# bentherien/point-cloud-reid

Hardware: AMD Instinct MI355X
Metric: siamese pair-comparisons/sec @1024 pts (higher is better)
Workload: dtype bf16x3

## Files before the change

point-cloud-reid_amd/csrc/attn_kernels_impl.h:

```cpp
#pragma once
#ifndef PCR_ATTN_PREC
#define PCR_ATTN_PREC 0
#endif
#include "tile_dense.h"
#include "wave_trace.h"

#include <stdio.h>

#include <initializer_list>
#include <vector>

namespace {
constexpr int kAPrec = PCR_ATTN_PREC;
struct AttnArgs {
  pcr_attn_params p;
  int dbg;
  int wpc;
  const int *live_count;
  int live_period, live_offset;
};

struct LiveWalk {
  unsigned n, period;
  long total;
  __device__ __forceinline__ long map(long v) const {
    const unsigned q = (unsigned)v / n;
    return (long)q * period + ((unsigned)v - q * n);
  }
};
__device__ __forceinline__ unsigned live_pairs(const AttnArgs &a) {
  int c = __builtin_amdgcn_readfirstlane(*a.live_count);
  c = c < 0 ? 0 : c;
  c -= a.live_offset;
  return (unsigned)(c < 0 ? 0 : (c > a.live_period ? a.live_period : c));
}
__device__ __forceinline__ LiveWalk live_walk(const AttnArgs &a) {
  LiveWalk w;
  w.n = live_pairs(a);
  w.period = (unsigned)a.live_period;
  const unsigned B = (unsigned)a.p.B, full = B / w.period, rem = B - full * w.period;
  w.total = (long)full * w.n + (rem < w.n ? rem : w.n);
  return w;
}
__device__ __forceinline__ bool live_cloud(const AttnArgs &a, unsigned b) {
  return b % (unsigned)a.live_period < live_pairs(a);
}

constexpr int kATraceWgs = 512, kATraceRecs = 24, kATraceMarks = 8;
using AttnTrace = WaveTrace<0, kATraceRecs, kATraceMarks, 2 * kATraceWgs>;
__device__ unsigned long long g_attn_trace[AttnTrace::kCap * AttnTrace::kWords];


__device__ __forceinline__ void pos_hidden(float *dst, int RP, const float *P, const float *w0,
                                           const float *b0, int d, int T) {
  for (int e = threadIdx.x; e < d * T; e += blockDim.x) {
    const int o = e / T, t = e - o * T;
    const float v = w0[o * 3] * P[t] + w0[o * 3 + 1] * P[RP + t] + w0[o * 3 + 2] * P[2 * RP + t] + b0[o];
    dst[o * RP + t] = fmaxf(v, 0.f);
  }
}

__device__ __forceinline__ void load_xyz3(float *P, int RP, const float *xyz, int L, int t0, int T) {
  for (int e = threadIdx.x; e < 3 * T; e += blockDim.x) {
    const int c = e / T, t = e - c * T;
    P[c * RP + t] = t0 + t < L ? xyz[(size_t)(t0 + t) * 3 + c] : 0.f;
  }
}

__device__ __forceinline__ void attn_kv_fold_write(const pcr_attn_params &p, const float *KVl, const float *s_kt, size_t b) {
  const int d = p.d, dh = d / p.nhead, ld = d + 1, tid = threadIdx.x;
  float *kv = p.kv + b * ((size_t)d * d + d);
  const int d_o = kThreads / d, d_dd = kThreads - d_o * d;
  int o = tid / d, dd = tid - o * d;
  int v0 = (dd / dh) * dh;
  for (int e = tid; e < d * d; e += kThreads, o += d_o, dd += d_dd) {
    if (dd >= d) {
      dd -= d;
      o++;
    }
    if (d_dd) v0 = (dd / dh) * dh;
    const float *wm = p.wmerge + (size_t)o * d + v0;
    const float *kr = KVl + dd * ld + v0;
    float m = 0.f;
#pragma unroll 8
    for (int v = 0; v < dh; v++) m += wm[v] * kr[v];
    if constexpr (kAPrec == 0) {
      const int kb = dd >> 3, rem = dd & 7;
      kv[(((size_t)kb * d + o) * 2 + (rem & 1)) * 4 + (rem >> 1)] = m;
    } else {
      const int s16 = dd >> 4, kk = dd & 15;
      const int hh = (kk >> 2) & 1, jj = (kk & 3) + ((kk >> 3) << 2);
      const size_t unit = (((size_t)s16 * (d >> 5) + (o >> 5)) * 2) * 64 + hh * 32 + (o & 31);
      const __bf16 hi = (__bf16)m;
      const __bf16 lo = (__bf16)(m - (float)hi);
      __bf16 *img = reinterpret_cast<__bf16 *>(kv);
      img[unit * 8 + jj] = hi;
      img[(unit + 64) * 8 + jj] = lo;
    }
  }
  __syncthreads();
  if (tid < d) kv[(size_t)d * d + tid] = s_kt[tid];
}

__device__ __forceinline__ void attn_kv_fold_mfma(const pcr_attn_params &p, const float *KVt, const float *s_kt, size_t b) {
  const int d = p.d, dh = d / p.nhead, ld = d + 1, tid = threadIdx.x;
  float *kv = p.kv + b * ((size_t)d * d + d);
  for (int hd = 0; hd < p.nhead; hd++) {
    const float *wm = p.wmerge_packed + (size_t)(hd * dh / 8) * d * 8;
    tile_dense(KVt + (size_t)(hd * dh) * ld + hd * dh, dh, ld, dh >> 5, wm, d, [&](float m, int o, int t) {
      const int dd = hd * dh + t;
      if constexpr (kAPrec == 0) {
        const int kb = dd >> 3, rem = dd & 7;
        kv[(((size_t)kb * d + o) * 2 + (rem & 1)) * 4 + (rem >> 1)] = m;
      } else {
        const int s16 = dd >> 4, kk = dd & 15;
        const int hh = (kk >> 2) & 1, jj = (kk & 3) + ((kk >> 3) << 2);
        const size_t unit = (((size_t)s16 * (d >> 5) + (o >> 5)) * 2) * 64 + hh * 32 + (o & 31);
        const __bf16 hi = (__bf16)m;
        const __bf16 lo = (__bf16)(m - (float)hi);
        __bf16 *img = reinterpret_cast<__bf16 *>(kv);
        img[unit * 8 + jj] = hi;
        img[(unit + 64) * 8 + jj] = lo;
      }
    });
  }
  __syncthreads();
  if (tid < d) kv[(size_t)d * d + tid] = s_kt[tid];
}

template <int TB, int NR, int WSEL, int NTW, bool BFP = false>
__device__ __forceinline__ void attn_kv_body(const AttnArgs &a) {
  constexpr int T = 32 * TB, RP = T + 1;
  constexpr int NPF = 4;
  extern __shared__ __attribute__((aligned(16))) float smem[];
  const pcr_attn_params &p = a.p;
  const int d = p.d, c2 = p.c2;
  float *XH = smem;
  float *KB = XH;
  float *VB = XH + d * RP;
  float *P = XH + (c2 + d) * RP;
  float *s_w0 = P + 3 * RP, *s_b0 = s_w0 + 3 * d;
  const int tail_a = (c2 + d + 3) * RP + 4 * d, tail_b = d * (d + 1) + d;
  float *s_ks = smem + (tail_a > tail_b ? tail_a : tail_b);
  const int tid = threadIdx.x, lane = tid & 63, wave = tid >> 6;
  const int l31 = lane & 31, h = lane >> 5;
  const size_t b = blockIdx.x;
  for (int e = tid; e < 3 * d; e += kThreads) s_w0[e] = p.pos0_w[e];
  for (int e = tid; e < d; e += kThreads) s_b0[e] = p.pos0_b[e];
  const float *feat = p.feat_k + b * c2 * p.Sk;
  const float *xyz = p.xyz_k + b * p.Sk * 3;
  const int nb = d >> 5, nT = nb * nb;
  const int dh = d / p.nhead;
  const float sk = (float)p.Sk;
  const float *bkv = p.bkv;

  f32x16 acc[NTW];
#pragma unroll
  for (int i = 0; i < NTW; i++)
#pragma unroll
    for (int r = 0; r < 16; r++) acc[i][r] = 0.f;
  int tile_ib[NTW];
#pragma unroll
// ... 28 lines not shown
        dst[2] = pf[u][2];
        dst[3] = pf[u][3];
      }
    }
  };
  const int nsplit = p.kv_splits > 1 ? p.kv_splits : 1;
  const int ntile = (p.Sk + T - 1) / T, tps = (ntile + nsplit - 1) / nsplit;
  const int t_lo = (int)blockIdx.y * tps * T;
  const int t_hi = (t_lo + tps * T) < p.Sk ? (t_lo + tps * T) : p.Sk;
  bool have = false;
  if (vec_ok && t_lo + T <= p.Sk && t_lo < t_hi) {
    fetch(t_lo);
    have = true;
  }
  for (int t0 = t_lo; t0 < t_hi; t0 += T) {
    const int valid = p.Sk - t0;
    if (have) stash();
    else load_tile(XH, RP, feat, c2, c2, p.Sk, t0, T);
    load_xyz3(P, RP, xyz, p.Sk, t0, T);
    __syncthreads();
    have = vec_ok && t0 + 2 * T <= p.Sk && t0 + T < t_hi;
    pos_hidden(XH + c2 * RP, RP, P, s_w0, s_b0, d, T);
    __syncthreads();
    auto kv_epi = [&](const f32x16 &acc, int cb, int tb, int l31, int h) {
      const int t = tb * 32 + l31;
      float *dst = XH + (cb * 32 + 4 * h) * RP + t;
      const bool live = t < valid;
      if (cb * 32 < d) {
#pragma unroll
        for (int r = 0; r < 16; r++) dst[((r & 3) + 8 * (r >> 2)) * RP] = live ? elu1(acc[r]) : 0.f;
      } else {
#pragma unroll
        for (int r = 0; r < 16; r++) dst[((r & 3) + 8 * (r >> 2)) * RP] = live ? acc[r] / sk : 0.f;
      }
    };
    auto kv_hook = [&]() { if (have) fetch(t0 + T); };
    if constexpr (BFP && kAPrec != 0 && WSEL != 0)
      tile_dense2p<kAPrec, TB, NR, WSEL, true>(XH, c2 + d, p.wkv_bf, 2 * d, true, kv_epi, bkv, nullptr, kv_hook);
    else
      tile_dense2<TB, NR, WSEL, true>(XH, c2 + d, p.wkv, 2 * d, true, kv_epi, bkv, nullptr, kv_hook);
    __syncthreads();
    {
      const float *row = KB + krow * RP;
      for (int t = kpart; t < T; t += kparts) ksum += row[t];
    }
#pragma unroll
    for (int it = 0; it < NTW; it++) {
      const int item = wave + 4 * it;
      if (item < nT) {
        const int ib = tile_ib[it], jb = item - ib * nb;
        const float *ap = KB + (ib * 32 + l31) * RP + h;
        const float *bp = VB + (jb * 32 + l31) * RP + h;
#pragma unroll 4
        for (int ks = 0; ks < T / 2; ks++)
          acc[it] = __builtin_amdgcn_mfma_f32_32x32x2f32(ap[2 * ks], bp[2 * ks], acc[it], 0, 0, 0);
      }
    }
    __syncthreads();
  }
  if (nsplit > 1) {
    float *part = p.kv_part + ((size_t)b * nsplit + blockIdx.y) * ((size_t)d * d + d);
    s_ks[tid] = ksum;
#pragma unroll
    for (int it = 0; it < NTW; it++) {
      const int item = wave + 4 * it;
      if (item < nT) {
        const int ib = tile_ib[it], jb = item - ib * nb;
#pragma unroll
        for (int r = 0; r < 16; r++)
          part[(size_t)(ib * 32 + (r & 3) + 8 * (r >> 2) + 4 * h) * d + jb * 32 + l31] = acc[it][r];
      }
    }
    __syncthreads();
    if (tid < d) {
      float s = 0.f;
      for (int pp = 0; pp < kparts; pp++) s += s_ks[pp * d + tid];
      part[(size_t)d * d + tid] = s;
    }
    return;
  }
  float *KVl = smem;
  const int ld = d + 1;
  const bool mfma_fold = p.wmerge_packed != nullptr && (dh & 31) == 0 && (d & 31) == 0;
  float *s_kt = smem + d * ld;
  s_ks[tid] = ksum;
#pragma unroll
  for (int it = 0; it < NTW; it++) {
    const int item = wave + 4 * it;
    if (item < nT) {
      const int ib = tile_ib[it], jb = item - ib * nb;
      const int v = jb * 32 + l31;
      const int hv = v / dh;
      const bool aligned = (dh & 31) == 0;
      const bool same_blk = (ib * 32) / dh == hv;
#pragma unroll
      for (int r = 0; r < 16; r++) {
        const int dd = ib * 32 + (r & 3) + 8 * (r >> 2) + 4 * h;
        const bool same = aligned ? same_blk : (dd / dh == hv);
        if (mfma_fold) KVl[v * ld + dd] = same ? acc[it][r] : 0.f;
        else KVl[dd * ld + v] = same ? acc[it][r] : 0.f;
      }
    }
  }
  __syncthreads();
  if (tid < d) {
    float s = 0.f;
    for (int pp = 0; pp < kparts; pp++) s += s_ks[pp * d + tid];
    s_kt[tid] = s;
  }
  if (mfma_fold) attn_kv_fold_mfma(p, KVl, s_kt, b);
  else attn_kv_fold_write(p, KVl, s_kt, b);
}

template <int TB, int NR, int WSEL, int NTW>
__global__ __launch_bounds__(kThreads) void attn_kv_kernel(AttnArgs a) {
  attn_kv_body<TB, NR, WSEL, NTW>(a);
}
template <int TB, int NR, int WSEL, int NTW>
__global__ __launch_bounds__(kThreads) __attribute__((amdgpu_waves_per_eu(3, 3))) void attn_kv_kernel_o3(AttnArgs a) {
  attn_kv_body<TB, NR, WSEL, NTW>(a);
}
template <int TB, int NR, int WSEL, int NTW>
__global__ __launch_bounds__(kThreads) __attribute__((amdgpu_waves_per_eu(3, 3))) void attn_kv_kernel_o3_live(AttnArgs a) {
  if (!live_cloud(a, blockIdx.x)) return;
  attn_kv_body<TB, NR, WSEL, NTW>(a);
}
template <int TB, int NR, int WSEL, int NTW, bool BFP = false>
__global__ __launch_bounds__(kThreads) __attribute__((amdgpu_waves_per_eu(2, 2))) void attn_kv_kernel_o2(AttnArgs a) {
  attn_kv_body<TB, NR, WSEL, NTW, BFP>(a);
}

constexpr int kKvsWaves = 8;
template <bool DIAG, bool BF, int XS = 4, bool ONEW = false, bool GATE = false>
__global__ __launch_bounds__(64 * kKvsWaves) __attribute__((amdgpu_waves_per_eu(2, 2)))
void attn_kv_stream64_kernel(AttnArgs a) {
  static_assert(BF || XS == 4, "the f32 form is c2 = 64 only");
  constexpr int D = 64, LD = D + 1, KVS = D * LD + D;
  constexpr int NKV = DIAG ? 2 : 4;
  constexpr int C2 = 16 * XS, WU = BF ? (XS + 4) * 512 : 4096, MINW = XS == 8 ? 4 : 2;
  extern __shared__ __attribute__((aligned(16))) float smem[];
  const pcr_attn_params &p = a.p;
  f32x4 *s_w = reinterpret_cast<f32x4 *>(smem);
  f32x4 *s_p0 = reinterpret_cast<f32x4 *>(smem + 4 * WU);
  float *s_bkv = smem + 4 * WU + 256;
  float *s_wm = s_bkv + 128;
  float *s_red = s_wm + D * LD;
  const int tid = threadIdx.x, lane = tid & 63, j = lane & 31, h = lane >> 5;
  const int wave = __builtin_amdgcn_readfirstlane(tid >> 6);
  LiveWalk lw{};
  if constexpr (GATE) {
    lw = live_walk(a);
    if ((long)blockIdx.x * (kKvsWaves / (ONEW ? 1 : 4)) >= lw.total) return;
  }
  {
    const f32x4 *src = reinterpret_cast<const f32x4 *>(BF ? p.wkv_bf : p.wkv);
    for (int e = tid; e < WU; e += 64 * kKvsWaves) s_w[e] = src[e];
    for (int e = tid; e < D * D; e += 64 * kKvsWaves) s_wm[(e >> 6) * LD + (e & 63)] = p.wmerge[e];
    if (tid < D) s_p0[tid] = f32x4{p.pos0_w[3 * tid], p.pos0_w[3 * tid + 1], p.pos0_w[3 * tid + 2], p.pos0_b[tid]};
    if (tid < 2 * D) s_bkv[tid] = p.bkv[tid];
  }
  __syncthreads();
  const int nblk = p.Sk >> 5;
  constexpr int kMaxWpc = 4;
  const int wpc = nblk < kMaxWpc ? nblk : kMaxWpc;
  int wpc2 = 1;
  while (wpc2 * 2 <= wpc) wpc2 *= 2;
  if (wpc2 < MINW) wpc2 = MINW;
  if constexpr (ONEW) wpc2 = 1;
  const int cpg = kKvsWaves / wpc2;
  const int cslot = wave / wpc2, wsub = wave - cslot * wpc2;
  const float inv_sk = 1.0f / (float)p.Sk;
  float bias[4];
#pragma unroll
  for (int cb = 0; cb < 4; cb++) bias[cb] = s_bkv[cb * 32 + j];
  const int dh = D / p.nhead;
  AttnTrace trace;
  if constexpr (kTraceBuild)
    trace.begin((a.dbg & 256) && lane == 0 && (wave == 0 || wave == 5) && blockIdx.x < kATraceWgs,
                g_attn_trace, 2 * blockIdx.x + (wave ? 1 : 0));
  const long nB = GATE ? lw.total : (long)p.B;
  for (long c0 = (long)blockIdx.x * cpg; c0 < nB; c0 += (long)gridDim.x * cpg) {
    const bool live = c0 + cslot < nB;
    const long b = GATE ? (live ? lw.map(c0 + cslot) : 0) : c0 + cslot;
    trace.mark(4);
    f32x16 kv[NKV];
#pragma unroll
    for (int i = 0; i < NKV; i++)
#pragma unroll
      for (int r = 0; r < 16; r++) kv[i][r] = 0.f;
    float ks0 = 0.f, ks1 = 0.f;
    if (live) {
      const float *feat = p.feat_k + (size_t)b * C2 * p.Sk;
      const float *xyz = p.xyz_k + (size_t)b * p.Sk * 3;
      const __amdgpu_buffer_rsrc_t rfeat =
          __builtin_amdgcn_make_buffer_rsrc(const_cast<float *>(feat), 0, C2 * p.Sk * 4, 0x00020000);
      for (int blk = wsub; blk < nblk; blk += wpc2) {
        asm volatile("" ::: "memory");
        trace.mark(0);
        const int t = blk * 32 + j;
        const float px = xyz[3 * t], py = xyz[3 * t + 1], pz = xyz[3 * t + 2];
        f32x16 acc[4];
        if constexpr (!BF) {
          float xr[64];
          {
            const int vo = (h * p.Sk + t) * 4;
#pragma unroll
            for (int s2 = 0; s2 < 32; s2++)
              xr[s2] = __builtin_bit_cast(float, __builtin_amdgcn_raw_buffer_load_b32(rfeat, vo, s2 * 2 * p.Sk * 4, 0));
          }
#pragma unroll
          for (int s2 = 0; s2 < 32; s2++) {
            const f32x4 w = s_p0[2 * s2 + h];
            const float v = w[0] * px + w[1] * py + w[2] * pz + w[3];
            xr[32 + s2] = fmaxf(v, 0.f);
          }
#pragma unroll
          for (int s2 = 0; s2 < 32; s2++) asm volatile("" : "+v"(xr[s2]));
#pragma unroll
          for (int cb = 0; cb < 4; cb++)
#pragma unroll
            for (int r = 0; r < 16; r++) acc[cb][r] = 0.f;
#pragma unroll
          for (int kb = 0; kb < 16; kb++) {
            f32x4 w[4];
#pragma unroll
            for (int cb = 0; cb < 4; cb++) w[cb] = s_w[((kb * 128 + cb * 32 + j) << 1) + h];
#pragma unroll
            for (int i = 0; i < 4; i++)
#pragma unroll
              for (int cb = 0; cb < 4; cb++)
                acc[cb] = __builtin_amdgcn_mfma_f32_32x32x2f32(xr[4 * kb + i], w[cb][i], acc[cb], 0, 0, 0);
          }
        } else {
          float xf[8 * XS];
          {
            const int vo = (4 * h * p.Sk + t) * 4;
#pragma unroll
            for (int e = 0; e < 8 * XS; e++) {
              const int ch = 16 * (e >> 3) + bf_kpos(0, e & 7);
              xf[e] = __builtin_bit_cast(float, __builtin_amdgcn_raw_buffer_load_b32(rfeat, vo, ch * p.Sk * 4, 0));
            }
          }
          bf16x8 ah[XS + 4], al[XS + 4];
#pragma unroll
          for (int s2 = 0; s2 < 4; s2++) {
            float hv[8];
#pragma unroll
            for (int e = 0; e < 8; e++) {
              const f32x4 w = s_p0[16 * s2 + bf_kpos(0, e) + 4 * h];
              const float v = w[0] * px + w[1] * py + w[2] * pz + w[3];
              hv[e] = relu_i(v);
            }
            bf_split8(hv, ah[XS + s2], al[XS + s2], true);
          }
#pragma unroll
          for (int e = 0; e < 8 * XS; e++) asm volatile("" : "+v"(xf[e]));
#pragma unroll
          for (int s2 = 0; s2 < XS; s2++) {
            float xv[8];
#pragma unroll
            for (int e = 0; e < 8; e++) xv[e] = xf[8 * s2 + e];
            bf_split8(xv, ah[s2], al[s2], true);
          }
#pragma unroll
          for (int cb = 0; cb < 4; cb++)
#pragma unroll
            for (int r = 0; r < 16; r++) acc[cb][r] = 0.f;
          trace.mark(1);
          const bf16x8 *wb = reinterpret_cast<const bf16x8 *>(s_w) + lane;
#pragma unroll
          for (int s2 = 0; s2 < XS + 4; s2++) {
            bf16x8 wh[4], wl[4];
#pragma unroll
            for (int cb = 0; cb < 4; cb++) {
              wh[cb] = wb[((s2 * 4 + cb) * 2) * 64];
              wl[cb] = wb[((s2 * 4 + cb) * 2 + 1) * 64];
            }
#pragma unroll
            for (int cb = 0; cb < 4; cb++) acc[cb] = __builtin_amdgcn_mfma_f32_32x32x16_bf16(ah[s2], wh[cb], acc[cb], 0, 0, 0);
#pragma unroll
            for (int cb = 0; cb < 4; cb++) acc[cb] = __builtin_amdgcn_mfma_f32_32x32x16_bf16(al[s2], wh[cb], acc[cb], 0, 0, 0);
#pragma unroll
            for (int cb = 0; cb < 4; cb++) acc[cb] = __builtin_amdgcn_mfma_f32_32x32x16_bf16(ah[s2], wl[cb], acc[cb], 0, 0, 0);
          }
        }
        trace.mark(2);
#pragma unroll
        for (int r = 0; r < 16; r++) {
          acc[0][r] = elu1(acc[0][r] + bias[0]);
          acc[1][r] = elu1(acc[1][r] + bias[1]);
          acc[2][r] = (acc[2][r] + bias[2]) * inv_sk;
          acc[3][r] = (acc[3][r] + bias[3]) * inv_sk;
          ks0 += acc[0][r];
          ks1 += acc[1][r];
        }
#pragma unroll
        for (int i = 0; i < NKV; i++) {
          const int ib = DIAG ? i : (i >> 1), jb = DIAG ? i : (i & 1);
#pragma unroll
          for (int r = 0; r < 16; r++) {
            if constexpr (ONEW) kv[i] = __builtin_amdgcn_mfma_f32_32x32x2f32(acc[2 + jb][r], acc[ib][r], kv[i], 0, 0, 0);
            else kv[i] = __builtin_amdgcn_mfma_f32_32x32x2f32(acc[ib][r], acc[2 + jb][r], kv[i], 0, 0, 0);
          }
        }
        trace.mark(3);
      }
    }
    trace.mark(5);
    ks0 += __shfl_xor(ks0, 32, 64);
    ks1 += __shfl_xor(ks1, 32, 64);
    if constexpr (ONEW) {
      if (live) {
        float *kvo = p.kv + (size_t)b * ((size_t)D * D + D);
        bf16x8 *img = reinterpret_cast<bf16x8 *>(kvo);
#pragma unroll
        for (int db = 0; db < 2; db++) {
          const int hd = (db * 32 + j) / dh;
#pragma unroll
          for (int ob = 0; ob < 2; ob++) {
            f32x16 m;
#pragma unroll
            for (int r = 0; r < 16; r++) m[r] = 0.f;
#pragma unroll
            for (int i = 0; i < NKV; i++) {
              const int ib = DIAG ? i : (i >> 1), jb = DIAG ? i : (i & 1);
              if (ib != db) continue;
              const float *wr = s_wm + (ob * 32 + j) * LD + jb * 32 + 4 * h;
#pragma unroll
              for (int r = 0; r < 16; r++) {
                const int vl = (r & 3) + 8 * (r >> 2);
                const float av = (jb * 32 + vl + 4 * h) / dh == hd ? kv[i][r] : 0.f;
                m = __builtin_amdgcn_mfma_f32_32x32x2f32(av, wr[vl], m, 0, 0, 0);
              }
            }
#pragma unroll
            for (int G = 0; G < 2; G++) {
              float v[8];
#pragma unroll
              for (int e = 0; e < 8; e++) v[e] = m[8 * G + e];
              bf16x8 hi, lo;
              bf_split8(v, hi, lo, true);
              const size_t unit = (((size_t)(db * 2 + G) * (D >> 5) + ob) * 2) * 64 + h * 32 + j;
              img[unit] = hi;
              img[unit + 64] = lo;
            }
          }
        }
        if (h == 0) {
          kvo[(size_t)D * D + j] = ks0;
          kvo[(size_t)D * D + 32 + j] = ks1;
        }
      }
      trace.mark(6);
      trace.mark(7);
      trace.next();
      continue;
    }
    float *KVl = s_red + cslot * KVS, *s_kt = KVl + D * LD;
    for (int round = 0; round < wpc2; round++) {
      if (wsub == round) {
#pragma unroll
        for (int i = 0; i < NKV; i++) {
          const int ib = DIAG ? i : (i >> 1), jb = DIAG ? i : (i & 1);
#pragma unroll
          for (int r = 0; r < 16; r++) {
            const int dd = ib * 32 + (r & 3) + 8 * (r >> 2) + 4 * h, v = jb * 32 + j;
            float *dst = KVl + dd * LD + v;
            *dst = round == 0 ? kv[i][r] : *dst + kv[i][r];
          }
        }
        if (h == 0) {
          s_kt[j] = round == 0 ? ks0 : s_kt[j] + ks0;
          s_kt[32 + j] = round == 0 ? ks1 : s_kt[32 + j] + ks1;
        }
      }
      __syncthreads();
    }
    trace.mark(6);
    if (live) {
      float *kvo = p.kv + (size_t)b * ((size_t)D * D + D);
      for (int ti = wsub; ti < 4; ti += wpc2) {
        const int ob = ti >> 1, db = ti & 1;
        const float *ap = s_wm + (ob * 32 + j) * LD + h;
        const float *bp = KVl + (db * 32 + j) * LD + h;
        const int hd = (db * 32 + j) / dh;
        f32x16 m;
#pragma unroll
        for (int r = 0; r < 16; r++) m[r] = 0.f;
        const int s_lo = DIAG ? db * 16 : 0, s_hi = DIAG ? db * 16 + 16 : 32;
        if constexpr (kAPrec == 0) {
#pragma unroll 4
          for (int s2 = s_lo; s2 < s_hi; s2++) {
            const float bv = bp[2 * s2];
            m = __builtin_amdgcn_mfma_f32_32x32x2f32(ap[2 * s2], (2 * s2 + h) / dh == hd ? bv : 0.f, m, 0, 0, 0);
          }
          const int dd = db * 32 + j;
#pragma unroll
          for (int r = 0; r < 16; r++) {
            const int o = ob * 32 + (r & 3) + 8 * (r >> 2) + 4 * h;
            const int kb = dd >> 3, rem = dd & 7;
            kvo[(((size_t)kb * D + o) * 2 + (rem & 1)) * 4 + (rem >> 1)] = m[r];
          }
        } else {
#pragma unroll 4
          for (int s2 = s_lo; s2 < s_hi; s2++) {
            const float bv = bp[2 * s2];
            m = __builtin_amdgcn_mfma_f32_32x32x2f32((2 * s2 + h) / dh == hd ? bv : 0.f, ap[2 * s2], m, 0, 0, 0);
          }
          bf16x8 *img = reinterpret_cast<bf16x8 *>(kvo);
#pragma unroll
          for (int G = 0; G < 2; G++) {
            float v[8];
#pragma unroll
            for (int e = 0; e < 8; e++) v[e] = m[8 * G + e];
            bf16x8 hi, lo;
            bf_split8(v, hi, lo, true);
            const size_t unit = (((size_t)(db * 2 + G) * (D >> 5) + ob) * 2) * 64 + h * 32 + j;
            img[unit] = hi;
            img[unit + 64] = lo;
          }
        }
      }
      for (int e = wsub * 64 + lane; e < D; e += 64 * wpc2) kvo[(size_t)D * D + e] = s_kt[e];
    }
    trace.mark(7);
    trace.next();
    __syncthreads();
  }
}

#if PCR_ATTN_PREC != 0
__global__ __launch_bounds__(64 * kKvsWaves) __attribute__((amdgpu_waves_per_eu(2, 4)))
void attn_kv_stream32_kernel(AttnArgs a) {
  constexpr int D = 32, LD = D + 1, KVS = D * LD + D;
  extern __shared__ __attribute__((aligned(16))) float smem[];
  const pcr_attn_params &p = a.p;
// ... 1502 lines not shown
  const bool wide = 2 * p.d > 128 || p.cout > 128 || p.cfinal > 128;
  if (tb == 4) return attn_plan_form(pl, PCR_ATTN_APPLY_TILE, {4, wide ? 2 : 1}, false, gated);
  if (tb == 2) return attn_plan_form(pl, PCR_ATTN_APPLY_TILE, {2, wide ? 2 : 1}, true, gated);
  int widest = 2 * p.d > p.cout ? 2 * p.d : p.cout;
  if (p.cfinal > widest) widest = p.cfinal;
  if (kAPrec != 0 && widest > 256) return PCR_ERR_INVALID;
  return attn_plan_form(pl, PCR_ATTN_APPLY_TILE, {1, widest > 512 ? 8 : (widest > 256 ? 4 : 2)}, false, gated);
}

static dim3 attn_grid(const AttnPlan &pl) {
  if (!pl.persistent) return dim3(pl.gx, pl.gy);
  const long cap = (long)pl.per_cu * pcr_cu_count();
  return dim3((unsigned)(pl.work < cap ? pl.work : cap));
}
template <auto KERN, auto KERN_LIVE>
static inline int attn_launch_g(const AttnPlan &pl, dim3 grid, hipStream_t st, const AttnArgs &a) {
  return pl.gated ? pcr_launch_lds<KERN_LIVE>(grid, dim3(pl.threads), pl.lds, st, a)
                  : pcr_launch_lds<KERN>(grid, dim3(pl.threads), pl.lds, st, a);
}

static int attn_launch_kv_tile(const AttnPlan &pl, const AttnArgs &a, hipStream_t st) {
  const dim3 g = attn_grid(pl), blk(pl.threads);
  if (pl.targ[0] == 2) return pcr_launch_lds<attn_kv_kernel<2, 1, 2, 1>>(g, blk, pl.lds, st, a);
  return pcr_launch_lds<attn_kv_kernel<1, 2, 0, 4>>(g, blk, pl.lds, st, a);
}
static int attn_launch_kv_tile_o3(const AttnPlan &pl, const AttnArgs &a, hipStream_t st) {
  return attn_launch_g<attn_kv_kernel_o3<2, 1, 1, 1>, attn_kv_kernel_o3_live<2, 1, 1, 1>>(pl, attn_grid(pl), st, a);
}
static int attn_launch_kv_tile_o2(const AttnPlan &pl, const AttnArgs &a, hipStream_t st) {
  const dim3 g = attn_grid(pl), blk(pl.threads);
  if (pl.targ[4]) return pcr_launch_lds<attn_kv_kernel_o2<1, 2, 1, 4, true>>(g, blk, pl.lds, st, a);
  return pcr_launch_lds<attn_kv_kernel_o2<1, 2, 1, 4>>(g, blk, pl.lds, st, a);
}
template <bool DIAG>
static int attn_launch_kv_stream64(const AttnPlan &pl, const AttnArgs &a, const AttnTune &t, hipStream_t st) {
  const dim3 g = attn_grid(pl);
  int rc = PCR_ERR_INVALID;
  if (!pl.targ[1])
    rc = attn_launch_g<attn_kv_stream64_kernel<DIAG, false>, attn_kv_stream64_kernel<DIAG, false, 4, false, true>>(pl, g, st, a);
#if PCR_ATTN_PREC != 0
  else if (pl.targ[2] == 8) rc = pcr_launch_lds<attn_kv_stream64_kernel<DIAG, true, 8>>(g, dim3(pl.threads), pl.lds, st, a);
  else if (pl.targ[3])
    rc = attn_launch_g<attn_kv_stream64_kernel<DIAG, true, 4, true>, attn_kv_stream64_kernel<DIAG, true, 4, true, true>>(pl, g, st, a);
  else rc = attn_launch_g<attn_kv_stream64_kernel<DIAG, true>, attn_kv_stream64_kernel<DIAG, true, 4, false, true>>(pl, g, st, a);
#endif
  if (pl.trace) attn_dump_trace(t.trace, "kv64", (int)g.x, (int)a.p.B, a.p.Sk);
  return rc;
}
#if PCR_ATTN_PREC != 0
static int attn_launch_kv_stream32(const AttnPlan &pl, const AttnArgs &a, hipStream_t st) {
  return pcr_launch_lds<attn_kv_stream32_kernel>(attn_grid(pl), dim3(pl.threads), pl.lds, st, a);
}
static int attn_launch_kv_stream128(const AttnPlan &pl, const AttnArgs &a, hipStream_t st) {
  const dim3 g = attn_grid(pl), blk(pl.threads);
  if (pl.targ[0] == 2) return pcr_launch_lds<attn_kv_stream128_kernel<2>>(g, blk, pl.lds, st, a);
  return pcr_launch_lds<attn_kv_stream128_kernel<4>>(g, blk, pl.lds, st, a);
}
#else
static int attn_launch_kv_wide(const AttnPlan &pl, const AttnArgs &a, hipStream_t st) {
  const dim3 g = attn_grid(pl), blk(pl.threads);
  if (pl.targ[0] == 2) return pcr_launch_lds<attn_kv_wide_kernel<2>>(g, blk, pl.lds, st, a);
  return pcr_launch_lds<attn_kv_wide_kernel<3>>(g, blk, pl.lds, st, a);
}
#endif

static int attn_launch_kv(const AttnPlan &pl, AttnArgs &a, const AttnTune &t, hipStream_t st) {
  int rc = PCR_ERR_INVALID;
  if (pl.family != PCR_ATTN_KV_WIDE) a.p.kv_splits = pl.splits;
  switch (pl.family) {
    case PCR_ATTN_KV_TILE: rc = attn_launch_kv_tile(pl, a, st); break;
    case PCR_ATTN_KV_TILE_O3: rc = attn_launch_kv_tile_o3(pl, a, st); break;
    case PCR_ATTN_KV_TILE_O2: rc = attn_launch_kv_tile_o2(pl, a, st); break;
    case PCR_ATTN_KV_STREAM64:
      return pl.targ[0] ? attn_launch_kv_stream64<true>(pl, a, t, st) : attn_launch_kv_stream64<false>(pl, a, t, st);
#if PCR_ATTN_PREC != 0
    case PCR_ATTN_KV_STREAM32: return attn_launch_kv_stream32(pl, a, st);
    case PCR_ATTN_KV_STREAM128: return attn_launch_kv_stream128(pl, a, st);
#else
    case PCR_ATTN_KV_WIDE: return attn_launch_kv_wide(pl, a, st);
#endif
    default: return PCR_ERR_INVALID;
  }
  if (rc != PCR_OK || !pl.fold) return rc;
  return pcr_launch_lds<attn_kv_fold_kernel>(dim3(a.p.B), dim3(pl.threads), pl.fold_lds, st, a);
}

static int attn_launch_apply_tile(const AttnPlan &pl, const AttnArgs &a, hipStream_t st) {
  const dim3 g = attn_grid(pl), blk(pl.threads);
  switch (pl.targ[0] * 10 + pl.targ[1]) {
    case 41: return pcr_launch_lds<attn_apply_kernel<4, 1>>(g, blk, pl.lds, st, a);
    case 42: return pcr_launch_lds<attn_apply_kernel<4, 2>>(g, blk, pl.lds, st, a);
    case 21: return attn_launch_g<attn_apply_kernel<2, 1>, attn_apply_kernel<2, 1, true>>(pl, g, st, a);
    case 22: return attn_launch_g<attn_apply_kernel<2, 2>, attn_apply_kernel<2, 2, true>>(pl, g, st, a);
    case 12: return pcr_launch_lds<attn_apply_kernel<1, 2>>(g, blk, pl.lds, st, a);
#if PCR_ATTN_PREC == 0
    case 14: return pcr_launch_lds<attn_apply_kernel<1, 4>>(g, blk, pl.lds, st, a);
    case 18: return pcr_launch_lds<attn_apply_kernel<1, 8>>(g, blk, pl.lds, st, a);
#endif
    default: return PCR_ERR_INVALID;
  }
}
#if PCR_ATTN_PREC != 0
template <bool QPOS>
static int attn_launch_apply_stream64(const AttnPlan &pl, const AttnArgs &a, const AttnTune &t, hipStream_t st) {
  const dim3 g = attn_grid(pl), blk(pl.threads);
  const int c1s = pl.targ[1], cf = pl.targ[2], nob = pl.targ[3], nd = pl.targ[4];
  int rc = PCR_ERR_INVALID;
  if (nd == 1) rc = pcr_launch_lds<attn_apply_stream64_kernel<QPOS, 2, 0, 1, 1>>(g, blk, pl.lds, st, a);
  else if (nob == 4) rc = pcr_launch_lds<attn_apply_stream64_kernel<QPOS, 4, 0, 4>>(g, blk, pl.lds, st, a);
  else if (c1s == 4 && cf && !pl.targ[5])
    rc = attn_launch_g<attn_apply_stream64_kernel<QPOS, 4, 4>, attn_apply_stream64_kernel<QPOS, 4, 4, 2, 2, false, true>>(pl, g, st, a);
  else if (c1s == 4 && !pl.targ[5])
    rc = attn_launch_g<attn_apply_stream64_kernel<QPOS, 4, 0>, attn_apply_stream64_kernel<QPOS, 4, 0, 2, 2, false, true>>(pl, g, st, a);
  else if constexpr (!QPOS) {
    if (pl.targ[5])
      return attn_launch_g<attn_apply_stream64_kernel<false, 4, 0, 2, 2, true>, attn_apply_stream64_kernel<false, 4, 0, 2, 2, true, true>>(pl, g, st, a);
    if (c1s == 1) rc = pcr_launch_lds<attn_apply_stream64_kernel<false, 1, 2, 1>>(g, blk, pl.lds, st, a);
    else if (cf) rc = pcr_launch_lds<attn_apply_stream64_kernel<false, 2, 4>>(g, blk, pl.lds, st, a);
    else rc = pcr_launch_lds<attn_apply_stream64_kernel<false, 2, 0>>(g, blk, pl.lds, st, a);
  }
  if (pl.trace) attn_dump_trace(t.trace, "apply64", (int)g.x, (int)a.p.B, a.p.Lq);
  return rc;
}
static int attn_launch_apply_stream128(const AttnPlan &pl, const AttnArgs &a, hipStream_t st) {
  const dim3 g = attn_grid(pl), blk(pl.threads);
  if (pl.targ[0] == 1) return pcr_launch_lds<attn_apply_stream128_kernel<1>>(g, blk, pl.lds, st, a);
  if (pl.targ[0] == 2) return pcr_launch_lds<attn_apply_stream128_kernel<2>>(g, blk, pl.lds, st, a);
  return pcr_launch_lds<attn_apply_stream128_kernel<4>>(g, blk, pl.lds, st, a);
}
#endif

static int attn_launch_apply(const AttnPlan &pl, const AttnArgs &a, const AttnTune &t, hipStream_t st) {
  (void)t;
  switch (pl.family) {
    case PCR_ATTN_APPLY_TILE: return attn_launch_apply_tile(pl, a, st);
#if PCR_ATTN_PREC != 0
    case PCR_ATTN_APPLY_STREAM64:
      return pl.targ[0] ? attn_launch_apply_stream64<true>(pl, a, t, st) : attn_launch_apply_stream64<false>(pl, a, t, st);
    case PCR_ATTN_APPLY_STREAM128: return attn_launch_apply_stream128(pl, a, st);
#endif
    default: return PCR_ERR_INVALID;
  }
}

static int attn_unit(const pcr_attn_params &p, const pcr_live *live, bool apply, AttnPlan *pl, bool launch, pcr_stream_t stream) {
  const AttnTune &t = attn_tune();
  *pl = AttnPlan();
  const int rc = apply ? attn_plan_apply(p, live != nullptr, t, pl) : attn_plan_kv(p, live != nullptr, t, pl);
  if (!launch) return rc;
  if (pl->arith >= 0) pcr_note_arith(pl->arith);
  if (rc != PCR_OK) return rc;
  AttnArgs a;
  a.p = p;
  a.dbg = pl->trace ? 256 : 0;
  a.wpc = pl->wpc;
  a.live_count = live ? live->count : nullptr;
  a.live_period = live ? live->period : 0;
  a.live_offset = live ? live->offset : 0;
  return apply ? attn_launch_apply(*pl, a, t, pcr_s(stream)) : attn_launch_kv(*pl, a, t, pcr_s(stream));
}

#if PCR_ATTN_PREC == 1
int pcr_attn_kv_bf3(const pcr_attn_params *pp, const pcr_live *live, AttnPlan *pl, bool launch, pcr_stream_t stream) {
  return attn_unit(*pp, live, false, pl, launch, stream);
}
int pcr_attn_apply_bf3(const pcr_attn_params *pp, const pcr_live *live, AttnPlan *pl, bool launch, pcr_stream_t stream) {
  return attn_unit(*pp, live, true, pl, launch, stream);
}
#else
int pcr_attn_kv_bf3(const pcr_attn_params *pp, const pcr_live *live, AttnPlan *pl, bool launch, pcr_stream_t stream);
int pcr_attn_apply_bf3(const pcr_attn_params *pp, const pcr_live *live, AttnPlan *pl, bool launch, pcr_stream_t stream);

static bool attn_bf(const pcr_attn_params &p, pcr_attn_params &q) {
  const int widest = 2 * p.d > p.cout ? (2 * p.d > p.cfinal ? 2 * p.d : p.cfinal) : (p.cout > p.cfinal ? p.cout : p.cfinal);
  if (p.precision == 0 || p.d > 128 || widest > 256 || !p.wq_bf || !p.wmlp0_bf || !p.wmlp2_bf ||
      (p.cfinal && !p.wfinal_bf))
    return false;
  q = p;
  q.wq = p.wq_bf; q.wmlp0 = p.wmlp0_bf; q.wmlp2 = p.wmlp2_bf; q.wfinal = p.wfinal_bf;
  return true;
}

PCR_EXPORT int pcr_attn_kv_splits(int B, int Sk, int d) {
  (void)B;
  if (Sk < 1 || d > 64) return 1;
  if ((d == 64 || d == 32) && (Sk & 31) == 0) return 1;
  const int ntile = (Sk + 63) / 64;
  return ntile >= 16 ? 4 : (ntile >= 8 ? 2 : 1);
}

static bool attn_pool_ok(const pcr_attn_params &p) {
  pcr_attn_params q;
  return aps64_shape(p) && p.c1 == 64 && p.cout == 64 && !p.cfinal && !p.q_pos && attn_bf(p, q);
}

static int attn_entry(const pcr_attn_params *pp, const pcr_live *live, bool apply, AttnPlan *pl, bool launch, pcr_stream_t stream) {
  if (!pp || attn_check(*pp)) return PCR_ERR_INVALID;
  if (apply && ((!pp->out && !pp->pool_out) || (pp->pool_out && !attn_pool_ok(*pp)))) return PCR_ERR_INVALID;
  if (live && !attn_live_shape(*pp)) return PCR_ERR_INVALID;
  if (launch && pp->B == 0) return PCR_OK;
  if (apply && pp->B > 65535) return PCR_ERR_INVALID;
  if (live && (!live->count || live->period < 1 || live->offset < 0)) return PCR_ERR_INVALID;
  pcr_attn_params q;
  if (attn_bf(*pp, q)) return apply ? pcr_attn_apply_bf3(&q, live, pl, launch, stream) : pcr_attn_kv_bf3(&q, live, pl, launch, stream);
  return attn_unit(*pp, live, apply, pl, launch, stream);
}

PCR_EXPORT int pcr_attn_kv_f32(const pcr_attn_params *pp, pcr_stream_t stream) {
  AttnPlan pl;
  return attn_entry(pp, nullptr, false, &pl, true, stream);
}
PCR_EXPORT int pcr_attn_kv_live_f32(const pcr_attn_params *pp, const pcr_live *live, pcr_stream_t stream) {
  AttnPlan pl;
  return attn_entry(pp, live, false, &pl, true, stream);
}
PCR_EXPORT int pcr_attn_apply_f32(const pcr_attn_params *pp, pcr_stream_t stream) {
  AttnPlan pl;
  return attn_entry(pp, nullptr, true, &pl, true, stream);
}
PCR_EXPORT int pcr_attn_apply_live_f32(const pcr_attn_params *pp, const pcr_live *live, pcr_stream_t stream) {
  AttnPlan pl;
  return attn_entry(pp, live, true, &pl, true, stream);
}
PCR_EXPORT int pcr_attn_live_ok(const pcr_attn_params *pp) {
  return (pp && !attn_check(*pp) && attn_live_shape(*pp)) ? 1 : 0;
}
PCR_EXPORT int pcr_attn_apply_pool_ok(const pcr_attn_params *pp) {
  return (pp && !attn_check(*pp) && attn_pool_ok(*pp)) ? 1 : 0;
}

PCR_EXPORT int pcr_attn_launch_form(const pcr_attn_params *pp, const pcr_live *live, int apply, int *form) {
  if (!form) return PCR_ERR_INVALID;
  AttnPlan pl;
  const int rc = attn_entry(pp, live, apply != 0, &pl, false, nullptr);
  if (rc != PCR_OK) return rc;
  for (int i = 0; i < PCR_ATTN_FORM_INTS; i++) form[i] = 0;
  form[0] = pl.arith;
  form[1] = pl.family;
  form[2] = pl.gated;
  form[3] = pl.ntarg;
  for (int i = 0; i < pl.ntarg; i++) form[4 + i] = pl.targ[i];
  if (!apply) {
    form[10] = pl.splits;
    form[11] = pl.fold;
    form[12] = pl.wpc;
  }
  form[13] = (int)pl.lds;
  return PCR_OK;
}
#endif
```

Before: 69640.

## Skip zero key-weight blocks for positional channels in KV projection

```diff
diff --git a/point-cloud-reid_amd/csrc/attn_kernels_impl.h b/point-cloud-reid_amd/csrc/attn_kernels_impl.h
--- a/point-cloud-reid_amd/csrc/attn_kernels_impl.h
+++ b/point-cloud-reid_amd/csrc/attn_kernels_impl.h
@@ -8,6 +8,7 @@
 #include <stdio.h>
 
 #include <initializer_list>
+#include <type_traits>
 #include <vector>
 
 namespace {
@@ -342,14 +343,28 @@
     lw = live_walk(a);
     if ((long)blockIdx.x * (kKvsWaves / (ONEW ? 1 : 4)) >= lw.total) return;
   }
+  static_assert(LD > D, "s_kz takes the pad column of s_wm's last row");
+  unsigned *s_kz = reinterpret_cast<unsigned *>(s_wm + (D - 1) * LD + D);
+  if (tid == 0) *s_kz = 0u;
+  __syncthreads();
   {
     const f32x4 *src = reinterpret_cast<const f32x4 *>(BF ? p.wkv_bf : p.wkv);
-    for (int e = tid; e < WU; e += 64 * kKvsWaves) s_w[e] = src[e];
+    unsigned nz = 0u;
+    for (int e = tid; e < WU; e += 64 * kKvsWaves) {
+      const f32x4 u = src[e];
+      s_w[e] = u;
+      const bool kz = BF ? ((e >> 9) >= XS && ((e >> 7) & 3) < 2) : ((e >> 8) >= 8 && ((e >> 1) & 127) < D);
+      typedef unsigned u32x4 __attribute__((ext_vector_type(4)));
+      const u32x4 ub = __builtin_bit_cast(u32x4, u);
+      if (kz) nz |= (ub[0] | ub[1] | ub[2] | ub[3]) & (BF ? 0x7FFF7FFFu : 0x7FFFFFFFu);
+    }
+    if (nz) atomicOr(s_kz, 1u);
     for (int e = tid; e < D * D; e += 64 * kKvsWaves) s_wm[(e >> 6) * LD + (e & 63)] = p.wmerge[e];
     if (tid < D) s_p0[tid] = f32x4{p.pos0_w[3 * tid], p.pos0_w[3 * tid + 1], p.pos0_w[3 * tid + 2], p.pos0_b[tid]};
     if (tid < 2 * D) s_bkv[tid] = p.bkv[tid];
   }
   __syncthreads();
+  const bool kfull = __builtin_amdgcn_readfirstlane((int)*s_kz) != 0 || (a.dbg & 512) != 0;
   const int nblk = p.Sk >> 5;
   constexpr int kMaxWpc = 4;
   const int wpc = nblk < kMaxWpc ? nblk : kMaxWpc;
@@ -410,16 +425,25 @@
           for (int cb = 0; cb < 4; cb++)
 #pragma unroll
             for (int r = 0; r < 16; r++) acc[cb][r] = 0.f;
-#pragma unroll
-          for (int kb = 0; kb < 16; kb++) {
+          auto project = [&](auto first, int kb) {
+            constexpr int CB0 = decltype(first)::value;
             f32x4 w[4];
 #pragma unroll
-            for (int cb = 0; cb < 4; cb++) w[cb] = s_w[((kb * 128 + cb * 32 + j) << 1) + h];
+            for (int cb = CB0; cb < 4; cb++) w[cb] = s_w[((kb * 128 + cb * 32 + j) << 1) + h];
 #pragma unroll
             for (int i = 0; i < 4; i++)
 #pragma unroll
-              for (int cb = 0; cb < 4; cb++)
+              for (int cb = CB0; cb < 4; cb++)
                 acc[cb] = __builtin_amdgcn_mfma_f32_32x32x2f32(xr[4 * kb + i], w[cb][i], acc[cb], 0, 0, 0);
+          };
+#pragma unroll
+          for (int kb = 0; kb < 8; kb++) project(std::integral_constant<int, 0>{}, kb);
+          if (kfull) {
+#pragma unroll
+            for (int kb = 8; kb < 16; kb++) project(std::integral_constant<int, 0>{}, kb);
+          } else {
+#pragma unroll
+            for (int kb = 8; kb < 16; kb++) project(std::integral_constant<int, 2>{}, kb);
           }
         } else {
           float xf[8 * XS];
@@ -431,9 +455,31 @@
               xf[e] = __builtin_bit_cast(float, __builtin_amdgcn_raw_buffer_load_b32(rfeat, vo, ch * p.Sk * 4, 0));
             }
           }
-          bf16x8 ah[XS + 4], al[XS + 4];
-#pragma unroll
-          for (int s2 = 0; s2 < 4; s2++) {
+#pragma unroll
+          for (int e = 0; e < 8 * XS; e++) asm volatile("" : "+v"(xf[e]));
+#pragma unroll
+          for (int cb = 0; cb < 4; cb++)
+#pragma unroll
+            for (int r = 0; r < 16; r++) acc[cb][r] = 0.f;
+          trace.mark(1);
+          const bf16x8 *wb = reinterpret_cast<const bf16x8 *>(s_w) + lane;
+          auto project = [&](auto first, int s2, const bf16x8 xh, const bf16x8 xl) {
+            constexpr int CB0 = decltype(first)::value;
+            bf16x8 wh[4], wl[4];
+#pragma unroll
+            for (int cb = CB0; cb < 4; cb++) {
+              wh[cb] = wb[((s2 * 4 + cb) * 2) * 64];
+              wl[cb] = wb[((s2 * 4 + cb) * 2 + 1) * 64];
+            }
+#pragma unroll
+            for (int cb = CB0; cb < 4; cb++) acc[cb] = __builtin_amdgcn_mfma_f32_32x32x16_bf16(xh, wh[cb], acc[cb], 0, 0, 0);
+#pragma unroll
+            for (int cb = CB0; cb < 4; cb++) acc[cb] = __builtin_amdgcn_mfma_f32_32x32x16_bf16(xl, wh[cb], acc[cb], 0, 0, 0);
+#pragma unroll
+            for (int cb = CB0; cb < 4; cb++) acc[cb] = __builtin_amdgcn_mfma_f32_32x32x16_bf16(xh, wl[cb], acc[cb], 0, 0, 0);
+          };
+          auto hidden = [&](auto first, int s2) {
+            asm volatile("" ::: "memory");
             float hv[8];
 #pragma unroll
             for (int e = 0; e < 8; e++) {
@@ -441,37 +487,25 @@
               const float v = w[0] * px + w[1] * py + w[2] * pz + w[3];
               hv[e] = relu_i(v);
             }
-            bf_split8(hv, ah[XS + s2], al[XS + s2], true);
-          }
-#pragma unroll
-          for (int e = 0; e < 8 * XS; e++) asm volatile("" : "+v"(xf[e]));
+            bf16x8 hh, hl;
+            bf_split8(hv, hh, hl, true);
+            project(first, XS + s2, hh, hl);
+          };
 #pragma unroll
           for (int s2 = 0; s2 < XS; s2++) {
             float xv[8];
 #pragma unroll
             for (int e = 0; e < 8; e++) xv[e] = xf[8 * s2 + e];
-            bf_split8(xv, ah[s2], al[s2], true);
+            bf16x8 xh, xl;
+            bf_split8(xv, xh, xl, true);
+            project(std::integral_constant<int, 0>{}, s2, xh, xl);
           }
-#pragma unroll
-          for (int cb = 0; cb < 4; cb++)
-#pragma unroll
-            for (int r = 0; r < 16; r++) acc[cb][r] = 0.f;
-          trace.mark(1);
-          const bf16x8 *wb = reinterpret_cast<const bf16x8 *>(s_w) + lane;
-#pragma unroll
-          for (int s2 = 0; s2 < XS + 4; s2++) {
-            bf16x8 wh[4], wl[4];
-#pragma unroll
-            for (int cb = 0; cb < 4; cb++) {
-              wh[cb] = wb[((s2 * 4 + cb) * 2) * 64];
-              wl[cb] = wb[((s2 * 4 + cb) * 2 + 1) * 64];
-            }
-#pragma unroll
-            for (int cb = 0; cb < 4; cb++) acc[cb] = __builtin_amdgcn_mfma_f32_32x32x16_bf16(ah[s2], wh[cb], acc[cb], 0, 0, 0);
-#pragma unroll
-            for (int cb = 0; cb < 4; cb++) acc[cb] = __builtin_amdgcn_mfma_f32_32x32x16_bf16(al[s2], wh[cb], acc[cb], 0, 0, 0);
-#pragma unroll
-            for (int cb = 0; cb < 4; cb++) acc[cb] = __builtin_amdgcn_mfma_f32_32x32x16_bf16(ah[s2], wl[cb], acc[cb], 0, 0, 0);
+          if (kfull) {
+#pragma unroll
+            for (int s2 = 0; s2 < 4; s2++) hidden(std::integral_constant<int, 0>{}, s2);
+          } else {
+#pragma unroll
+            for (int s2 = 0; s2 < 4; s2++) hidden(std::integral_constant<int, 2>{}, s2);
           }
         }
         trace.mark(2);
@@ -2280,7 +2314,7 @@
   if (rc != PCR_OK) return rc;
   AttnArgs a;
   a.p = p;
-  a.dbg = pl->trace ? 256 : 0;
+  a.dbg = (pl->trace ? 256 : 0) | (pcr_tune_int("PCR_ATTN_KV_FULL") ? 512 : 0);
   a.wpc = pl->wpc;
   a.live_count = live ? live->count : nullptr;
   a.live_period = live ? live->period : 0;
```

Result: faster. 70800 (median of 6 runs) (+1.7%).
